# 001cat/pySurfInv

Measured on AMD Instinct MI355X. Metric: layered-model dispersion forward solves/sec (20 periods), higher is better.
Workload: dtype f32 (root search, Love group velocity) + f64 (Rayleigh eigenfunction state)

## Files before the change

### pysurfinv_amd/csrc/surfdisp_kernels.hip

```cpp
#include <hip/hip_runtime.h>
#include <stdint.h>
#include <type_traits>
#include <atomic>
#include "surfdisp_internal.h"

#include "surfdisp_k_common.h"
#include "surfdisp_k_prep.h"
#include "surfdisp_k_secular.h"
#include "surfdisp_k_rows.h"

namespace sd {

enum { ST_SCAN = 0, ST_REFINE = 1, ST_ELLIP = 2, ST_DONE = 3, ST_NEVILL = 4, ST_WREF = 5, ST_WEND = 6, ST_NEVILL0 = 7 };


template <int KIND, int G, bool INDEP, bool FAST = false, bool EXACT = false>
__device__ __forceinline__ void phase_body(const PhaseArgs &A)
{
    extern __shared__ float w_lds[];
    constexpr int S = SD_PHASE_BLOCK / G;
    constexpr int NFK = (KIND == 1) ? NFW_LOVE : NFW;
    constexpr int LS = lds_ls(S, NFK);
    const int tid = threadIdx.x;
#ifdef SD_WAVECLOCK
    const unsigned long long wclk0 = __builtin_amdgcn_s_memrealtime();
    const unsigned long long wcyc0 = __builtin_readcyclecounter();
    unsigned long long wcyc_eval = 0, wcyc_build = 0, wcyc_pre = 0, wpasses = 0;
    unsigned long long wsec[3] = {0, 0, 0}, wcyc_lean = 0, wn_lean = 0;
    unsigned long long wn_scan = 0, wn_refine = 0, wn_nevill = 0, wn_ellip = 0, wn_idle = 0, wtrip = 0, wlanelayers = 0, wlanes = 0;
#endif
    const int lane = tid & 63;
    const int slot = tid / G;
    const int j = tid % G;
    const int tbase = lane - j;
    const unsigned long long tmask =
        (G == 64) ? ~0ull : (((1ull << (G & 63)) - 1ull) << tbase);
    const int Lcap = A.Lmax, B = A.B, P = A.P;
    long tg = (long)blockIdx.x * S + slot;
    bool team_valid = INDEP ? (tg < (long)B * P) : (tg < B);
    if (EXACT) {
        team_valid = tg < (long)(*A.fb_count);
        tg = team_valid ? (long)A.fb_list[tg] : 0;
    }
    const int b = INDEP ? (int)(tg % B) : (int)tg;
    const int k_own = INDEP ? (int)(tg / B) : 0;
    float *wq = w_lds + slot;
    constexpr bool ELL_HERE = EXACT || (G < 4);
    const bool want_ratio = ELL_HERE && (KIND == 2) && (A.ratio != nullptr);
    constexpr bool OVERLAP = false;
    float *nvx = w_lds + (size_t)((!EXACT && G >= 4 && A.overlap != 0) ? 2 : 1) * LS * Lcap + (size_t)slot * 24, *nvy = nvx + 12;
    const float *__restrict__ mrow = A.msrc + (size_t)b * A.ms_b;
    const size_t msf = (size_t)A.ms_f, msi = (size_t)A.ms_i;
#define M_AT(f, i) mrow[(size_t)(f) * msf + (size_t)(i) * msi]

    int n = 0, st = ST_DONE;
    if (team_valid) { n = A.nl[b]; if (n >= 2) st = ST_SCAN; }

    int k = k_own, nsolved = 0, mm_carry = n, mm_frozen = n, sub = 0, passes = 0;
    int nflat_cur = n;
    float T = 1.0f, b1top = 0.0f;
    float p0c = 0.0f, p0d = 0.0f;
    float cb = 0.0f, db = 0.0f;
    float croot = 0.0f, r12 = 0.0f;
    int p0mm = 0;
    bool p0ok = false;
    bool first = true;
    int status = SURFDISP_OK;
    constexpr int FSTRIDE = (FAST && G <= 4) ? SD_CERT_STRIDE : 4;
    static_assert(!(FAST && EXACT), "the exact fallback walks every grid point");
    constexpr bool CERT = FAST && (G >= 2) && (G <= 8);
    int p0Kp = 0x40000000;
    bool coarse = false;
    int fine_left = 1;
    float q0c = 0.0f, q0d = 0.0f; int q0mm = 0; [[maybe_unused]] bool q0ok = false;
    [[maybe_unused]] float p0phi = 0.0f;
    bool ell_pend = false;
    int nv_nev = 1, nv_m = 1, nv_ic = 0;
    bool defer = false;
    bool ell_flag = false;
    const float ell_c2min = (want_ratio && !EXACT && team_valid && A.ovf != nullptr && A.ell_ambig != 0.0f)
                                ? __expf(0.25f * A.ovf[2 * (size_t)B + b]) / A.ell_gmax : 0.0f;

    auto build = [&](int nflat) {
        const float lnT = logf(1.0f / T);
        for (int i = j; i < nflat; i += G) {
            const bool hs = (i == nflat - 1);
            LayerRaw r;
            r.a_ref = M_AT(F_VP, i); r.b_ref = M_AT(F_VS, i); r.rho_ref = M_AT(F_RHO, i);
            r.qs = M_AT(F_QS, i);
            r.dif = hs ? 0.0f : M_AT(F_DIF, i); r.qqq = hs ? 0.0f : M_AT(F_QQQ, i);
            r.dfl = hs ? 0.0f : M_AT(F_DFL, i);
            r.hsf = hs ? M_AT(F_HSF, i) : 0.0f; r.hsr = hs ? M_AT(F_HSR, i) : 0.0f;
            const LayerV v = layer_derive(r, lnT, hs);
            W_B(i) = v.b; W_R(i) = v.rho; W_D(i) = v.d;
            if (KIND == 1 && !EXACT) W_IR(i) = wk_ilove(v.rho, v.b);
            else if (i == 0 || EXACT) W_IR(i) = wk_irho(v.rho);
            if (KIND == 2) {
                W_IA2(i) = EXACT ? v.a : wk_ia2(v.a);
                W_IB2(i) = wk_ib2(v.b);
            }
        }
        if (KIND == 2 && !EXACT) {
            __builtin_amdgcn_wave_barrier();
            __builtin_amdgcn_fence(__ATOMIC_RELEASE, "wavefront");
            __builtin_amdgcn_fence(__ATOMIC_ACQUIRE, "wavefront");
            const int top = nflat < n ? nflat : n - 1;
            for (int i = 1 + j; i <= top; i += G) W_IR(i) = wk_rat(W_R(i - 1), W_R(i));
        }
        __builtin_amdgcn_wave_barrier();
        __builtin_amdgcn_fence(__ATOMIC_RELEASE, "wavefront");
        __builtin_amdgcn_fence(__ATOMIC_ACQUIRE, "wavefront");
    };

    float dtot = 0.0f;
    auto bracket_phase = [&](float c1, float c2, int mm) -> float {
        const float om = 6.2831853f * __builtin_amdgcn_rcpf(T);
        const float i1 = __builtin_amdgcn_rcpf(c1 * c1), i2 = __builtin_amdgcn_rcpf(c2 * c2);
        const float sq = 1.001f * om * sqrt_hw(fmaxf(i1 - i2, 0.0f));
        if (sq * dtot * ((KIND == 2) ? 2.0f : 1.0f) <= A.phimulti) return 0.0f;
        float dosc = 0.0f;
        for (int i = j; i < mm - 1; i += G) {
            const float d = W_D(i);
            if (KIND == 2) dosc += ((W_IB2(i) > i2) ? d : 0.0f) + ((W_IA2(i) > i2) ? d : 0.0f);
            else           dosc += (W_B(i) < c2) ? d : 0.0f;
        }
#pragma unroll
        for (int d = G >> 1; d > 0; d >>= 1) dosc += __shfl_xor(dosc, d);
        if (sq * dosc <= A.phimulti) return 0.0f;
        float sum = 0.0f;
        for (int i = j; i < mm - 1; i += G) {
            const float od = om * W_D(i);
            const float ib2 = (KIND == 2) ? W_IB2(i) : W_IR(i) * W_R(i);
            sum += od * (sqrt_hw(fmaxf(ib2 - i2, 0.0f)) - sqrt_hw(fmaxf(ib2 - i1, 0.0f)));
            if (KIND == 2) {
                const float ia2 = W_IA2(i);
                sum += od * (sqrt_hw(fmaxf(ia2 - i2, 0.0f)) - sqrt_hw(fmaxf(ia2 - i1, 0.0f)));
            }
        }
#pragma unroll
        for (int d = G >> 1; d > 0; d >>= 1) sum += __shfl_xor(sum, d);
        return fabsf(sum);
    };

    auto entry_overflow_risk = [&](float c_lo) -> bool {
        if (EXACT || !team_valid) return false;
        if (KIND == 1) {
            const float bb = W_B(0);
            if (!(bb > c_lo)) return !(c_lo > 0.0f && T > 0.0f);
            const float q0 = 6.2831853f * __builtin_amdgcn_rcpf(c_lo * T) * W_D(0) *
                             sqrt_hw(fmaxf(1.0f - c_lo * c_lo * __builtin_amdgcn_rcpf(bb * bb), 0.0f));
            return !(q0 < 76.0f);
        }
        const float hthick = A.ovf[b], lnrho2 = A.ovf[(size_t)B + b], lng4 = A.ovf[2 * (size_t)B + b];
        const float c_hi = W_B(mm_carry - 1) + 0.31f;
        const float lnmag = 12.566371f * hthick / (c_lo * T) + lnrho2 + 4.0f * __logf(c_hi) +
                            fmaxf(lng4 - 8.0f * __logf(c_lo), 0.0f);
        return !(lnmag < 84.0f);
    };

    bool nodrop = false;
    auto no_drop_possible = [&](float c_lo) -> bool {
        float dsum = 0.0f;
        for (int i = j; i < n; i += G) dsum += W_D(i);
#pragma unroll
        for (int d = G >> 1; d > 0; d >>= 1) dsum += __shfl_xor(dsum, d);
        dtot = dsum;
        return dsum * 1.00001f <= FACT * c_lo * T;
    };

    if (st != ST_DONE) {
        T = A.per[k];
        for (int i = j; i < Lcap; i += G) { W_IR(i) = 0.0f; W_B(i) = 0.0f; W_R(i) = 0.0f; W_D(i) = 0.0f; if (KIND == 2) { W_IA2(i) = 0.0f; W_IB2(i) = 0.0f; } }
        build(n);
        b1top = W_B(0);
        const bool water = M_AT(F_VS, 0) < 0.1f;
        const int il = water ? 1 : 0;
        const float b_corr = M_AT(F_QS, il) * logf(1.0f / T) / PI_REF;
        float qq = M_AT(F_VS, il);
        if (KIND == 2) qq = 0.9f * qq;
        p0c = qq * (1.0f + b_corr);
        if (water) p0c = 0.5f;
        first = true;
        nodrop = no_drop_possible(p0c);
        defer = (!EXACT && A.strict != 0) || entry_overflow_risk(p0c);
        if (CERT) coarse = nodrop;
    }

    int wprio = -1;
    const bool LOCK = !EXACT && (INDEP ? A.lockstep >= 2 : A.lockstep != 0);
#ifdef SD_DEBUG_TRIALS
    constexpr bool LEAN = false;
#else
    constexpr bool LEAN = !FAST && !EXACT && !INDEP && (G == 2);
#endif
#ifdef SD_NO_GUARD_HANDBACK
    constexpr bool LEAN_BHS = false;
#else
    constexpr bool LEAN_BHS = LEAN && (KIND == 2);
#endif
    auto nevill_start = [&]() {
        nv_ic = 0; nv_nev = 1; nv_m = 1;
        croot = (p0c + cb) / 2.0f;
        st = (KIND == 1 && !EXACT) ? ST_NEVILL0 : ST_NEVILL;
        sub = 0;
        if (!EXACT && j == 0 && A.amb_count) atomicAdd(A.amb_count, 1);
    };
    while (__any(st != ST_DONE)) {
#ifdef SD_WAVECLOCK
        const unsigned long long wp0 = __builtin_readcyclecounter();
#endif
        if (!INDEP && A.balance) {
            const int kw = __builtin_amdgcn_readfirstlane(k);
            const int pr = 3 - min(3, (4 * kw) / max(P, 1));
            if (pr != wprio) {
                wprio = pr;
                if (pr == 3) __builtin_amdgcn_s_setprio(3);
                else if (pr == 2) __builtin_amdgcn_s_setprio(2);
                else if (pr == 1) __builtin_amdgcn_s_setprio(1);
                else __builtin_amdgcn_s_setprio(0);
            }
        }
        const bool lean = LEAN && A.scan_general == 0 && __all(st == ST_SCAN || st == ST_WREF || st == ST_DONE);
        float cj = 1.0f;
        int mmj = 2, start = 1;
        bool eval = (st != ST_DONE) && (st != ST_WREF) && (st != ST_WEND);
        const int js = (OVERLAP && ell_pend && st == ST_SCAN) ? j - 2 : j;
        if (st == ST_SCAN) {
            const int nadd = (CERT && coarse) ? FSTRIDE * (first ? js : js + 1) : (first ? js : js + 1);
            cj = p0c;
            if (CERT) {
#pragma unroll
                for (int i = 0; i < FSTRIDE * G; ++i) if (i < nadd) cj = cj + DC;
            } else {
#pragma unroll
                for (int i = 0; i < G; ++i) if (i < nadd) cj = cj + DC;
            }
            mmj = nodrop ? (n < 2 ? 2 : n) : drop_layers(wq, LS, S, n, cj, T);
        } else if (st == ST_NEVILL0) {
            const bool hi = (G == 1) ? (sub != 0) : ((j & 1) != 0);
            cj = hi ? cb : p0c; mmj = hi ? mm_frozen : p0mm;
        } else if (st == ST_NEVILL) {
            cj = croot; mmj = mm_frozen;
        } else if (st == ST_REFINE) {
            const float w = cb - p0c;
            cj = p0c + (float)(j + 1) * (w * (1.0f / (float)(G + 1)));
            if (G <= 4 && G > 1 && p0ok && w > 16.0f * CLUSTER_DC) {
                float ts = -p0d * w * __builtin_amdgcn_rcpf(db - p0d);
                const float off = (G == 4) ? ((j == 0) ? -4.0f : (j == 1) ? -1.0f : (j == 2) ? 1.0f : 4.0f)
                                           : ((j == 0) ? -1.5f : 1.5f);
                const float half = ((G == 4) ? 4.0f : 1.5f) * CLUSTER_DC;
                ts = fminf(fmaxf(ts, half + CLUSTER_DC), w - half - CLUSTER_DC);
                if (ts == ts) cj = p0c + (ts + off * CLUSTER_DC);
            }
            mmj = mm_frozen;
        } else if (st == ST_ELLIP) {
            cj = croot; mmj = mm_frozen;
            start = (G == 1) ? 2 + sub : 2 + j;
            eval = (G == 1) || (j < 2);
        }
        float val = 0.0f, phj = 0.0f;
        int kcj = 0; bool kuncj = false;
#ifdef SD_WAVECLOCK
        const unsigned long long we0 = __builtin_readcyclecounter();
        wcyc_pre += we0 - wp0;
        ++wpasses;
        {
            const unsigned long long lead = __ballot(j == 0);
            wn_scan += __popcll(__ballot(st == ST_SCAN) & lead); wn_refine += __popcll(__ballot(st == ST_REFINE) & lead);
            wn_nevill += __popcll(__ballot(st == ST_NEVILL) & lead); wn_ellip += __popcll(__ballot(st == ST_ELLIP) & lead);
            wn_idle += __popcll(__ballot(st == ST_DONE || st == ST_WREF || st == ST_WEND) & lead);
            int mx = eval ? mmj : 0, sm = eval ? mmj : 0;
            for (int d = 32; d > 0; d >>= 1) { mx = max(mx, __shfl_xor(mx, d)); sm += __shfl_xor(sm, d); }
            wtrip += mx; wlanelayers += sm; wlanes += __popcll(__ballot(eval));
        }
#endif
        float vmag = 0.0f;
        [[maybe_unused]] float bhsj = 0.0f;
        if (eval) {
            const bool want_mag = want_ratio && st == ST_ELLIP;
            if (KIND == 2) val = EXACT ? delta_rayleigh_ref(wq, LS, S, mmj, cj, T, start)
                                       : delta_rayleigh<(G != 2) && !FAST, CERT, (G <= 16)>(wq, LS, S, mmj, cj, T, start, phj, &vmag, want_mag, &kcj, &kuncj, coarse,
                                                                                                            LEAN_BHS ? &bhsj : nullptr
#ifdef SD_WAVECLOCK
                                                                                                            , wsec
#endif
                                                                                                            );
            else if (!EXACT && (st == ST_NEVILL || st == ST_NEVILL0)) val = delta_love_ref_body(wq, LS, S, mmj, cj, T);
            else           val = EXACT ? delta_love_ref(wq, LS, S, mmj, cj, T)
                                       : delta_love<CERT, (G <= 16)>(wq, LS, S, mmj, cj, T, phj, kcj, kuncj, coarse);
        }
        const bool ell_amb = !EXACT && want_ratio && eval && st == ST_ELLIP && A.ell_ambig != 0.0f &&
                             (A.ell_ambig < 0.0f || fabsf(val) < A.ell_ambig * vmag ||
                              cj * cj < ell_c2min);
#ifdef SD_WAVECLOCK
        const unsigned long long wl0 = __builtin_readcyclecounter();
        wcyc_eval += wl0 - we0;
#endif
        if (lean) {
            const bool scan = (st == ST_SCAN);
            auto negnan = [](float x) { return signbit(x) && !(x != x); };
            float oc = cj, od = val; int omm = mmj;
            float sc = p0c, sv_ = p0d; int smm = p0mm;
            if (G == 2) {
                oc = pair_swap(cj); od = pair_swap(val); omm = pair_swap(mmj);
                sc = oc; sv_ = od; smm = omm;
            } else if (G > 2) {
                const int lm1 = (lane + 63) & 63;
                sc = __shfl(cj, lm1); sv_ = __shfl(val, lm1); smm = __shfl(mmj, lm1);
            }
            const float pc = (j == 0) ? p0c : sc, pd = (j == 0) ? p0d : sv_;
            const int pmm = (j == 0) ? p0mm : smm;
            const bool has_prev = !(first && j == 0);
            const bool cross = has_prev && (negnan(val) != negnan(pd));
            bool guard = false;
            if (scan && has_prev && !cross) {
                if constexpr (LEAN_BHS) guard = (cj < 0.8f * b1top) || !(cj < bhsj + 0.3f);
                else                    guard = (cj < 0.8f * b1top) || !(cj < W_B(mmj - 1) + 0.3f);
            }
            const unsigned long long em = __ballot(scan && (cross || guard)) & tmask;
            const int fl = em ? (__ffsll((long long)em) - 1) : -1;
            const int q = (fl < 0) ? tbase + G - 1 : fl;
            const bool q_cross = ((__ballot(cross) >> q) & 1ull) != 0ull;
            float q_c, q_d, q_pc, q_pd;
            int q_mm, q_pmm;
            if (G == 1) {
                q_c = cj; q_d = val; q_mm = mmj; q_pc = pc; q_pd = pd; q_pmm = pmm;
            } else if (G == 2) {
                const bool mine = (q == lane), q_lo = (q == tbase);
                q_c = mine ? cj : oc; q_d = mine ? val : od; q_mm = mine ? mmj : omm;
                q_pc = q_lo ? p0c : ((j == 0) ? cj : oc);
                q_pd = q_lo ? p0d : ((j == 0) ? val : od);
                q_pmm = q_lo ? p0mm : ((j == 0) ? mmj : omm);
            } else {
                q_c = __shfl(cj, q); q_d = __shfl(val, q); q_mm = __shfl(mmj, q);
                q_pc = __shfl(pc, q); q_pd = __shfl(pd, q); q_pmm = __shfl(pmm, q);
            }
            if (scan && ((__ballot(scan && !fin(val)) & tmask) != 0ull)) defer = true;
            bool failed = false;
            if (scan) {
                ++passes;
                if (fl >= 0 && q_cross) {
                    p0c = q_pc; p0d = q_pd; cb = q_c; db = q_d; mm_frozen = q_mm; p0mm = q_pmm;
                    p0ok = (q_pmm == q_mm);
                    passes = 0;
                    st = LOCK ? ST_WREF : ST_REFINE;
                    if (!LOCK && bracket_phase(p0c, cb, mm_frozen) > A.phimulti) nevill_start();
                } else if (fl >= 0) {
                    failed = true;
                } else {
                    p0c = q_c; p0d = q_d; p0mm = q_mm; first = false;
                    if (passes > 100000) failed = true;
                }
            }
            if (defer) {
                if (j == 0) A.fb_list[atomicAdd(A.fb_count, 1)] = (int)tg;
                defer = false; st = ST_DONE; failed = false;
            }
            if (failed) {
                status = (k == 0) ? SURFDISP_NOROOT : SURFDISP_PARTIAL;
                st = ST_DONE;
            }
            if (LOCK && !__any(st == ST_SCAN) && st == ST_WREF) {
                st = ST_REFINE;
                if (bracket_phase(p0c, cb, mm_frozen) > A.phimulti) nevill_start();
            }
#ifdef SD_WAVECLOCK
            wcyc_lean += __builtin_readcyclecounter() - wl0; ++wn_lean;
#endif
            continue;
        }
        const int lm1 = (lane + 63) & 63;
        const float sc = __shfl(cj, lm1), sv_ = __shfl(val, lm1);
        const float pc = (j == 0) ? p0c : sc;
        const float pd = (j == 0) ? p0d : sv_;
        const int smm = __shfl(mmj, lm1);
        const int pmm = (j == 0) ? p0mm : smm;
        const int kpk = CERT ? ((kcj + 4096) | (kuncj ? 0x40000000 : 0)) : 0;
        const int sKp = CERT ? __shfl(kpk, lm1) : 0;
        const int pKp = (j == 0) ? p0Kp : sKp;
        const bool searching = ((st == ST_SCAN) || (st == ST_REFINE)) ;
        const bool has_prev = !((st == ST_SCAN) && first && (js == 0));
        auto negnan = [](float x) { return signbit(x) && !(x != x); };
        const bool cross = has_prev && (negnan(val) != negnan(pd));
#ifdef SD_DEBUG_TRIALS
        if (A.B == 1 && eval && k == SD_DEBUG_TRIALS && cj > SD_DEBUG_CMIN)
            printf("k %d pass %d st %d lane %d c %.7f val % .6e mm %d count %d unsafe %d coarse %d | p0c %.7f p0d % .4e cb %.7f db % .4e\n", k, passes, st, j, cj, val, mmj, kcj, (int)kuncj, (int)coarse, p0c, p0d, cb, db);
#endif
        bool guard = false;
        if (st == ST_SCAN && has_prev && !cross)
            guard = (cj < 0.8f * b1top) || !(cj < W_B(mmj - 1) + 0.3f);
        bool uncert = false, back0 = false;
        if (CERT) {
            if (coarse && st == ST_SCAN) {
                const bool near_hs = !(cj < W_B(mmj - 1) - 2.0f * (float)FSTRIDE * DC);
                const bool low_guard = (pc + DC) < 0.8f * b1top;
                uncert = has_prev && (near_hs || low_guard || !((pmm == mmj) && fin(pd) && fin(val) && !kuncj && (pKp == kpk)));
            }
        }
        const bool ev = searching && (cross || guard || uncert);
        const unsigned long long em = __ballot(ev) & tmask;
        const int fl = em ? (__ffsll((long long)em) - 1) : -1;
        const int src = (fl < 0) ? tbase : fl;
        const float e_c = __shfl(cj, src), e_d = __shfl(val, src);
        const float e_pc = __shfl(pc, src), e_pd = __shfl(pd, src);
        const int e_mm = __shfl(mmj, src);
        const int e_pmm = __shfl(pmm, src);
        const int l_mm = __shfl(mmj, tbase + G - 1);
        const int e_cross = __shfl((int)cross, src);
        const int t_back0 = CERT ? __shfl((int)back0, tbase) : 0;
        const int lastl = tbase + G - 1;
        const float l_c = __shfl(cj, lastl), l_d = __shfl(val, lastl);
        const float l_phi = CERT ? __shfl(phj, lastl) : 0.0f;
        const int l_Kp = CERT ? __shfl(kpk, lastl) : 0;
        const int e_pKp = CERT ? __shfl(pKp, src) : 0;
        float v0 = 0.0f, v1 = 0.0f;
        if (__any((st == ST_ELLIP) | (st == ST_NEVILL) | (st == ST_NEVILL0))) { v0 = __shfl(val, tbase); v1 = __shfl(val, (G > 1) ? tbase + 1 : tbase); }
        float e_nc = 0.0f, e_nd = 0.0f, pl_c = 0.0f, pl_d = 0.0f, e_ppc = 0.0f, e_ppd = 0.0f, e_n2c = 0.0f, e_n2d = 0.0f,
              pl2_c = 0.0f, pl2_d = 0.0f;
        int pl_mm = 0;
        if (CERT || __any(st == ST_REFINE)) {
            const int nxt = (src < lastl) ? src + 1 : lastl;
            e_nc = __shfl(cj, nxt); e_nd = __shfl(val, nxt);
            const int pl = (G > 1) ? lastl - 1 : lastl;
            pl_c = __shfl(cj, pl); pl_d = __shfl(val, pl);
            if (CERT) pl_mm = __shfl(mmj, pl);
            const int lm2s = (src - 2 >= tbase) ? src - 2 : tbase;
            e_ppc = __shfl(cj, lm2s); e_ppd = __shfl(val, lm2s);
            const int nx2 = (src + 2 <= lastl) ? src + 2 : lastl;
            e_n2c = __shfl(cj, nx2); e_n2d = __shfl(val, nx2);
            const int pl2 = (G > 2) ? lastl - 2 : lastl;
            pl2_c = __shfl(cj, pl2); pl2_d = __shfl(val, pl2);
        }
        const bool had_ell = OVERLAP && ell_pend && (st == ST_SCAN);

        bool solved = false, failed = false;
        bool fatal = false, multi = false;
        if (!EXACT) {
            const bool nonfin = ((__ballot(eval && !fin(val)) & tmask) != 0ull);
            if (st != ST_DONE && nonfin) defer = true;
            if (st == ST_REFINE && passes == 0) {
                const int ncross = __popcll(__ballot(searching && cross) & tmask) + ((negnan(l_d) != negnan(db)) ? 1 : 0);
                multi = ncross >= 2;
            }
        }
        if (CERT && st == ST_SCAN && coarse) {
            ++passes;
            if (fl >= 0) {
                p0c = e_pc; p0d = e_pd; p0mm = e_pmm;
                if (CERT) p0Kp = e_pKp;
                const bool e_back = (fl == tbase) && (t_back0 != 0);
                if (e_back) { p0c = q0c; p0d = q0d; p0mm = q0mm; }
                coarse = false; fine_left = (e_cross && !e_back) ? FSTRIDE : 2 * FSTRIDE; q0ok = false;
                if (CERT) { fine_left = FSTRIDE; first = false; }
            } else {
                q0c = pl_c; q0d = pl_d; q0mm = pl_mm; q0ok = true;
                p0c = l_c; p0d = l_d; p0mm = l_mm; p0phi = l_phi;
                if (CERT) { p0Kp = l_Kp; first = false; }
            }
        } else if (st == ST_SCAN) {
            ++passes;
            if (fl >= 0 && e_cross) {
                p0c = e_pc; p0d = e_pd; cb = e_c; db = e_d; mm_frozen = e_mm; p0mm = e_pmm;
                p0ok = (e_pmm == e_mm);
                passes = 0;
                st = LOCK ? ST_WREF : ST_REFINE;
                if (EXACT || (!LOCK && bracket_phase(p0c, cb, mm_frozen) > A.phimulti)) nevill_start();
            } else if (fl >= 0) {
                failed = true;
            } else {
                p0c = l_c; p0d = l_d; p0mm = l_mm; first = false;
                if (CERT) p0Kp = l_Kp;
                if (CERT) { p0phi = l_phi; q0d = pl_d; q0mm = pl_mm; }
                if (passes > 100000) failed = true;
                if (CERT) {
                    fine_left -= had_ell ? G - 2 : G;
                    if (fine_left <= 0 && nodrop) { coarse = true; q0ok = false; }
                    if (CERT && coarse) first = true;
                }
            }
        } else if (!EXACT && st == ST_REFINE && multi) {
            nv_ic = 0; nv_nev = 1; nv_m = 1;
            croot = (p0c + cb) / 2.0f;
            st = (KIND == 1) ? ST_NEVILL0 : ST_NEVILL;
            sub = 0;
        } else if (st == ST_NEVILL0) {
            if (G == 1) { if (sub == 0) { p0d = val; sub = 1; } else { db = val; st = ST_NEVILL; } }
            else { p0d = v0; db = v1; st = ST_NEVILL; }
        } else if (st == ST_NEVILL) {
#pragma clang fp contract(off)
            auto sg = [](float x) { return (signbit(x) && !(x != x)) ? -1.0f : 1.0f; };
            auto sgsub = [&](float a, float bq) {
                const float r = a - bq;
                if (r != r) return ((a != a) || (bq != bq)) ? 1.0f : -1.0f;
                return signbit(r) ? -1.0f : 1.0f;
            };
            float c1 = p0c, c2 = cb, d1 = p0d, d2 = db, c3 = croot;
            const float d3 = v0;
            nv_ic = nv_ic + 1;
            bool fin_ = false;
            if (!(nv_ic < 50)) fatal = true;
            else {
                bool bis;
                if (c1 - c3 <= 0.0f) bis = (c2 - c3 <= 0.0f);
                else bis = !(c2 - c3 < 0.0f);
                if (!bis) {
                    const float s13s = sgsub(d1, d3), s32s = sgsub(d3, d2);
                    if (sg(d3) * sg(d1) <= 0.0f) { c2 = c3; d2 = d3; } else { c1 = c3; d1 = d3; }
                    if (fabsf(c1 - c2) - 0.1e-5f <= 0.0f) fin_ = true;
                    else {
                        if (s13s != s32s) nv_nev = 0;
                        const float ss1 = fabsf(d1), s1 = 0.1f * ss1, ss2 = fabsf(d2), s2 = 0.1f * ss2;
                        if (s1 > ss2 || s2 > ss1) bis = true;
                        else if (nv_nev == 0) bis = true;
                        else {
                            int m = nv_m;
                            if (nv_nev == 2) { nvx[m + 1] = c3; nvy[m + 1] = d3; }
                            else { nvx[1] = c1; nvy[1] = d1; nvx[2] = c2; nvy[2] = d2; m = 1; }
                            const float ym1 = nvy[m + 1];
                            for (int kk = 1; kk <= m; ++kk) {
                                const int jn = m - kk + 1;
                                const float yj = nvy[jn];
                                if (fabsf(ym1 - yj) <= 0.1e-7f) { bis = true; break; }
                                nvx[jn] = (-yj * nvx[jn + 1] + ym1 * nvx[jn]) / (ym1 - yj);
                            }
                            if (!bis) { c3 = nvx[1]; nv_nev = 2; nv_m = (m + 1 > 10) ? 10 : m + 1; }
                        }
                    }
                }
                if (!fin_ && bis) { c3 = (c1 + c2) / 2.0f; nv_nev = 1; nv_m = 1; }
                p0c = c1; p0d = d1; cb = c2; db = d2; croot = c3;
            }
            if (fin_) {
                if (croot <= W_B(mm_frozen - 1)) {
                    if (want_ratio) { st = ST_ELLIP; sub = 0; } else solved = true;
                } else failed = true;
            }
        } else if (st == ST_REFINE) {
            float tc, td;
            bool tok = true;
            float uc = 0.0f, ud = 0.0f;
            bool uok = false;
            const float oa = p0c, oda = p0d, ob = cb, odb = db;
            const bool oaok = p0ok;
            if (fl >= 0) {
                if (fl != tbase) p0ok = true;
                p0c = e_pc; p0d = e_pd; cb = e_c; db = e_d;
                if (fl < lastl) { tc = e_nc; td = e_nd; } else { tc = ob; td = odb; }
                if (fl >= tbase + 2) { uc = e_ppc; ud = e_ppd; uok = true; }
                else if (fl == tbase + 1) { uc = oa; ud = oda; uok = oaok; }
                else if (fl + 2 <= lastl) { uc = e_n2c; ud = e_n2d; uok = true; }
                else if (fl + 1 == lastl) { uc = ob; ud = odb; uok = true; }
            } else {
                p0c = l_c; p0d = l_d; p0ok = true;
                if (G > 1) { tc = pl_c; td = pl_d; } else { tc = oa; td = oda; tok = oaok; }
                if (G > 2) { uc = pl2_c; ud = pl2_d; uok = true; }
            }
            {
                const float w = cb - p0c, sx = tc - p0c;
                const float fm = fmaxf(fabsf(p0d), fabsf(db));
                const int fex = (fm > 0.0f && fin(fm)) ? __builtin_amdgcn_frexp_expf(fm) : 0;
                const float f0 = ldexpf(p0d, -fex), f1 = ldexpf(db, -fex), f2 = ldexpf(td, -fex);
                ud = ldexpf(ud, -fex);
                auto qt = [](float a, float bq) { return a * __builtin_amdgcn_rcpf(bq); };
                float ts = qt(-f0 * w, f1 - f0);
                float t = qt(w * (f0 * f2), (f1 - f0) * (f1 - f2)) + qt(sx * (f0 * f1), (f2 - f0) * (f2 - f1));
                if (!(ts >= 0.0f)) ts = 0.0f;
                if (!(ts <= w)) ts = w;
                if (!p0ok) ts = 0.5f * w;
                const bool inside = p0ok && tok && (t >= 0.0f) && (t <= w);
                auto bends = [&](float xs, float fs) {
                    const float dm = f1 - f0;
                    const float dn = (xs > w) ? fs - f1 : f0 - fs, hn = (xs > w) ? xs - w : 0.0f - xs;
                    return !(fabsf(dn * w - dm * hn) <= 0.25f * fabsf(dm * hn));
                };
                const bool smooth = inside && !bends(sx, f2);
                bool agree = smooth && (fabsf(t - ts) <= A.atol);
                if (smooth && !agree && uok && !bends(uc - p0c, ud)) {
                    const float sx2 = uc - p0c, f3 = ud;
                    const float t2 = qt(w * (f0 * f3), (f1 - f0) * (f1 - f3)) + qt(sx2 * (f0 * f1), (f3 - f0) * (f3 - f1));
                    agree = (t2 >= 0.0f) && (t2 <= w) && (fabsf(t - t2) <= A.atol);
                }
                ++passes;
                bool accept = !(w > 1.0e-6f) || passes > 64;
                if (!accept && !(w > A.wtol) && agree) {
                    accept = !(W_B(mm_frozen - 1) <= cb * 1.000001f);
#ifdef SD_COUNT_KINK
                    if (j == 0 && A.amb_count && !accept) atomicAdd(A.amb_count + 1, 1);
#endif
                }
                if (accept) {
                    croot = p0c + (inside ? t : ts);
                    if (p0c >= 16.0f) fatal = true;
                    else if (croot <= W_B(mm_frozen - 1)) {
                        if (want_ratio) { st = ST_ELLIP; sub = 0; } else solved = true;
                    } else failed = true;
                }
            }
        } else if (st == ST_ELLIP) {
            if ((__ballot(ell_amb) & tmask) != 0ull) ell_flag = true;
            if (G == 1) {
                if (sub == 0) { r12 = val; sub = 1; }
                else { r12 = 0.5f * val / r12; solved = true; }
            } else {
                r12 = 0.5f * v1 / v0;
                solved = true;
            }
        }
        if (!EXACT && defer) {
            if (j == 0) A.fb_list[atomicAdd(A.fb_count, 1)] = (int)tg;
            defer = false; st = ST_DONE; solved = false; failed = false; fatal = false;
        }
        if (fatal) {
            nsolved = 0; k = 0; status = SURFDISP_NUMERIC; st = ST_DONE; ell_pend = false; solved = false; failed = false;
        }
        if (failed) {
            status = (k == 0) ? SURFDISP_NOROOT : SURFDISP_PARTIAL;
            st = ST_DONE;
        }
        if (LOCK) {
            if (solved) { st = ST_WEND; solved = false; }
            if (!__any(st == ST_SCAN) && st == ST_WREF) {
                st = ST_REFINE;
                if (bracket_phase(p0c, cb, mm_frozen) > A.phimulti) nevill_start();
            }
            if (!__any(st == ST_SCAN || st == ST_WREF || st == ST_REFINE || st == ST_NEVILL || st == ST_NEVILL0 || st == ST_ELLIP) && st == ST_WEND)
                solved = true;
        }
#ifdef SD_WAVECLOCK
        const unsigned long long wb0 = __builtin_readcyclecounter();
#endif
        if (solved) {
            if (j == 0) {
                A.c[(size_t)k * B + b] = croot;
                if (want_ratio) A.ratio[(size_t)k * B + b] = r12;
                if (A.hist) A.hist[(size_t)k * B + b] = EXACT ? (int)(0x80000000u | (unsigned)nflat_cur | ((unsigned)mm_frozen << 16))
                                                              : (nflat_cur | (mm_frozen << 16) | (ell_flag ? 0x40000000 : 0));
            }
            ell_flag = false;
            nsolved = ++k;
            if (INDEP || k >= P) { st = ST_DONE; }
            else {
                T = A.per[k];
                mm_carry = mm_frozen;
#ifdef SD_DEBUG_TRIALS
                if (A.B == 1 && j == 0) printf("period %d starts: previous root %.7f, layers rebuilt for T = %.4f: %d of %d\n", k, croot, T, mm_carry, n);
#endif
                build(mm_carry);
                nflat_cur = mm_carry;
                b1top = W_B(0);
                p0c = 0.90f * croot;
                p0d = 0.0f; p0mm = 0; p0ok = false; first = true; passes = 0;
                coarse = false; fine_left = 1; q0ok = false;
                st = ST_SCAN;
                nodrop = no_drop_possible(p0c);
                defer = entry_overflow_risk(p0c);
                if (CERT) coarse = nodrop;
            }
        }
#ifdef SD_WAVECLOCK
        wcyc_build += __builtin_readcyclecounter() - wb0;
#endif
    }
#ifdef SD_WAVECLOCK
    if (!EXACT && A.wclk && (threadIdx.x & 63) == 0) {
        const size_t w = (size_t)blockIdx.x * (SD_PHASE_BLOCK / 64) + (threadIdx.x >> 6);
        unsigned long long *o = A.wclk + 24 * w;
        o[0] = wclk0; o[1] = __builtin_amdgcn_s_memrealtime();
        o[2] = __builtin_readcyclecounter() - wcyc0; o[3] = wcyc_eval;
        o[4] = wcyc_build; o[5] = wpasses; o[6] = wcyc_pre;
        o[7] = wn_scan; o[8] = wn_refine; o[9] = wn_nevill; o[10] = wn_ellip; o[11] = wn_idle;
        o[12] = wtrip; o[13] = wlanelayers; o[14] = wlanes; o[15] = wsec[0];
        o[16] = wsec[1]; o[17] = wsec[2]; o[18] = wcyc_lean; o[19] = wn_lean;
    }
#endif
    if (INDEP) {
        if (team_valid && j == 0 && n >= 2 && status != SURFDISP_OK) {
            A.c[(size_t)k_own * B + b] = 0.0f;
            atomicMin(&A.nsolved[b], status == SURFDISP_NUMERIC ? -1 : k_own);
        }
        return;
    }
    if (team_valid && j == 0) {
        if (n < 2) status = SURFDISP_BADMODEL;
        for (int q = nsolved; q < P; ++q) A.c[(size_t)q * B + b] = 0.0f;
        A.nsolved[b] = nsolved;
        if (A.status) A.status[b] = status;
    }
#undef M_AT
}

template <int KIND, int G, bool INDEP, bool FAST = false, bool EXACT = false>
__global__ __launch_bounds__(SD_PHASE_BLOCK) void surfdisp_phase_kernel(PhaseArgs A)
{
    phase_body<KIND, G, INDEP, FAST, EXACT>(A);
}

__global__ __launch_bounds__(256) void surfdisp_ellip_kernel(EllipArgs A)
{
    const size_t idx = (size_t)blockIdx.x * blockDim.x + threadIdx.x;
    const int B = A.B, P = A.P;
    if (idx >= (size_t)B * P) return;
    const int b = (int)(idx % B), k = (int)(idx / B);
    const int n = A.nl[b];
    if (n < 2 || k >= A.nsolved[b]) return;
    const int hk = A.hist[idx];
    if (hk < 0) return;
    if (A.only_flagged && !(hk & 0x40000000)) return;
    const int mmf = (hk >> 16) & 0x3fff;
    const size_t fs = (size_t)A.Lmax * B;
    const float c = A.c[idx], T = A.per[k];
    struct Replay { int kk, nflat; float lnT; };
    const Replay r0{k, hk & 0xffff, logf(1.0f / T)};
    auto layer = [&](int i, Replay &r) -> LayerV {
        while (r.nflat <= i && r.kk > 0) {
            --r.kk;
            const int h = A.hist[(size_t)r.kk * B + b];
            r.nflat = (h < 0) ? n : (h & 0xffff);
            r.lnT = logf(1.0f / A.per[r.kk]);
        }
        return layer_derive(layer_load(A.mdl, fs, (size_t)i * B + b), r.lnT, i == r.nflat - 1);
    };
    const int last = mmf - 1;
    float v2 = 0.0f, v3 = 0.0f;
    bool exact = A.only_flagged != 0;
    if (!exact) {
        const RTrial t = ray_trial(c, T);
        int kk = k;
        int nflat = hk & 0xffff;
        float lnT = r0.lnT;
        RState s2{}, s3{};
        float phi = 0.0f, rho_prev = 0.0f;
        RLyr y{};
        float rho_i = 0.0f;
        for (int i = 0; i <= last; ++i) {
            while (nflat <= i && kk > 0) {
                --kk;
                const int h = A.hist[(size_t)kk * B + b];
                nflat = (h < 0) ? n : (h & 0xffff);
                lnT = logf(1.0f / A.per[kk]);
            }
            const LayerV v = layer_derive(layer_load(A.mdl, fs, (size_t)i * B + b), lnT, i == nflat - 1);
            rho_prev = rho_i;
            rho_i = v.rho;
            y.sv = v.b; y.d = v.d;
            y.ia2 = wk_ia2(v.a);
            y.ib2 = wk_ib2(v.b);
            y.rat = (i > 0) ? wk_rat(rho_prev, rho_i) : 0.0f;
            if (i == 0) {
                const float irho0 = wk_irho(rho_i);
                s2 = ray_start(t, 2, irho0);
                s3 = ray_start(t, 3, irho0);
                if (last >= 1) { ray_step<true>(s2, t, y, 2, phi); ray_step<true>(s3, t, y, 3, phi); }
            } else if (i < last) {
                ray_step<false>(s2, t, y, 2, phi);
                ray_step<false>(s3, t, y, 3, phi);
            }
        }
        const float rp = (last >= 1) ? rho_prev : 0.0f;
        float m2 = 0.0f, m3 = 0.0f;
        v2 = ray_close(s2, t, y, rho_i, rp, 2, &m2); v3 = ray_close(s3, t, y, rho_i, rp, 3, &m3);
        const float b2max = A.ovf ? 0.5f * __expf(0.25f * A.ovf[2 * (size_t)B + b]) : 0.0f;
        exact = (A.ell_ambig < 0.0f) ||
                ((A.ell_ambig > 0.0f) && (fabsf(v2) < A.ell_ambig * m2 || fabsf(v3) < A.ell_ambig * m3 || 2.0f * b2max > A.ell_gmax * c * c));
    }
    if (exact) {
        Replay r = r0;
        v2 = delta_rayleigh_ref_gen([&](int m) { const LayerV v = layer(m, r); return RefLyr{v.a, v.b, v.rho, v.d}; }, mmf, c, T, 2);
        r = r0;
        v3 = delta_rayleigh_ref_gen([&](int m) { const LayerV v = layer(m, r); return RefLyr{v.a, v.b, v.rho, v.d}; }, mmf, c, T, 3);
        if (A.amb_count) atomicAdd(A.amb_count + 1, 1);
    }
    A.ratio[idx] = 0.5f * v3 / v2;
}

struct Drop { int hs_layer; int nreg_hs; };

template <int KIND>
SD_HD __forceinline__ Drop drop_group(const float *__restrict__ mdl, size_t fs, int B, int b,
                                           int n, float lnT, float c, float T, int ndiv, bool water,
                                           float div)
{
    const float dmax = FACT * T * c;
    float sum = 0.0f;
    Drop r; r.hs_layer = n - 1; r.nreg_hs = 0;
    LayerRaw nraw = layer_load(mdl, fs, (size_t)b);
    for (int jl = 0; jl < n; ++jl) {
        const LayerRaw raw = nraw;
        if (jl + 1 < n) nraw = layer_load(mdl, fs, (size_t)(jl + 1) * B + b);
        const LayerV v = layer_derive(raw, lnT, jl == n - 1);
        if (!(c < v.b)) continue;
        if (jl == n - 1) break;
        const int nsub = (jl == 0 && water) ? 1 : ndiv;
        const float dsub = (ndiv > 1 && !(jl == 0 && water)) ? v.d / div : v.d;
        for (int s = 0; s < nsub; ++s) sum = sum + dsub;
        if (!(sum > dmax)) continue;
        const LayerV nx = layer_derive(nraw, lnT, jl + 1 == n - 1);
        bool lower, equal;
        if (KIND == 2) {
            lower = (nx.a < v.a) || (nx.a == v.a && nx.b < v.b);
            equal = (nx.a == v.a) && (nx.b == v.b);
        } else {
            lower = nx.b < v.b;
            equal = nx.b == v.b;
        }
        if (lower) { r.hs_layer = jl; r.nreg_hs = nsub - 1; break; }
        if (equal) continue;
        r.hs_layer = jl + 1; r.nreg_hs = 0; break;
    }
    return r;
}

#define SD_NO_DROP_SLACK 1.0e-4f
SD_HD __forceinline__ bool group_no_cut(const float *__restrict__ mdl, size_t fs, int B, int b, int n, float c, float T)
{
    float tot = 0.0f;
    for (int jl = 0; jl + 1 < n; ++jl) tot = tot + fabsf(mdl[F_DFL * fs + (size_t)jl * B + b]);
    return tot * (1.0f + SD_NO_DROP_SLACK) <= FACT * T * c;
}
template <int KIND>
SD_HD __forceinline__ Drop drop_or_none(const float *__restrict__ mdl, size_t fs, int B, int b,
                                             int n, float lnT, float c, float T, int ndiv, bool water,
                                             float div)
{
#ifndef SD_NO_DROP_SHORTCUT
    if (group_no_cut(mdl, fs, B, b, n, c, T)) return Drop{n - 1, 0};
#endif
    return drop_group<KIND>(mdl, fs, B, b, n, lnT, c, T, ndiv, water, div);
}

struct KOut {
    float *b;
    size_t stride;
    ptrdiff_t off_a, off_r;
    int raw;
    SD_HD void put(int i, float vb, float va, float vr) const
    {
        float *q = b + (size_t)i * stride;
        *q = vb;
        if (off_a) *reinterpret_cast<float *>(reinterpret_cast<char *>(q) + off_a) = va;
        if (off_r) *reinterpret_cast<float *>(reinterpret_cast<char *>(q) + off_r) = vr;
    }
};
struct EOut {
    float *p;
    size_t stride, plane;
    SD_HD void put(int i, float ur, float uz, float tz, float tr) const
    {
        float *q = p + (size_t)i * stride;
        q[0] = ur; q[plane] = uz; q[2 * plane] = tz; q[3 * plane] = tr;
    }
    SD_HD void put2(int i, float ut, float tq) const
    {
        float *q = p + (size_t)i * stride;
        q[0] = ut; q[plane] = tq;
    }
};
struct EUnit { float div; int hs; float i0, i1, i2; };
struct K3 { float b, a, r; };
struct Chain { float dbdb, dadb, dada, rfac; };
SD_HD __forceinline__ Chain chain_of(const LayerRaw &r, float lnT, bool is_halfspace, bool raw)
{
    if (raw) return Chain{1.0f, 0.0f, 1.0f, 1.0f};
    const float qsq = r.qs * lnT / PI_REF;
    const float qpq = qsq * 1.33333333f * (r.b_ref * r.b_ref) / (r.a_ref * r.a_ref);
    const float vfac = is_halfspace ? r.hsf : r.dif;
    Chain ch;
    ch.dbdb = (1.0f + qsq) * vfac;
    ch.dadb = 2.66666667f * qsq * (r.b_ref / r.a_ref) * vfac;
    ch.dada = (1.0f - qpq) * vfac;
    ch.rfac = is_halfspace ? r.hsr : r.qqq;
    return ch;
}
struct KC { float b1, b2, a, r; };
SD_HD __forceinline__ KC kern_coef(const LayerRaw &raw, const LayerV &v, float lnT, bool is_halfspace, float cw, bool rawc)
{
    const Chain ch = chain_of(raw, lnT, is_halfspace, rawc);
    const float rc2 = 2.0f * v.rho * cw;
    return KC{rc2 * v.b * ch.dbdb, rc2 * v.a * ch.dadb, rc2 * v.a * ch.dada, cw * ch.rfac / v.rho};
}
typedef double KR;
SD_HD __forceinline__ K3 kern_layer_rayleigh(const KC &kc, float rho, float xlamb, float xmu, float wvno, float wvnosq,
                                             float omegsq, KR dmmr, KR dmmz, KR drsz, KR dzsr, KR smmz, KR smmr)
{
    const KR two = 2, k2 = wvnosq, tk = 2.0f * wvno;
    const KR dldl = -k2 * dmmr + tk * drsz - smmz;
    const KR dldm = -k2 * (two * dmmr + dmmz) - tk * dzsr - (two * smmz + smmr);
    const KR dldr = (KR)omegsq * (dmmr + dmmz);
    return K3{(float)((KR)kc.b1 * (dldm - two * dldl) + (KR)kc.b2 * dldl), (float)((KR)kc.a * dldl),
              (float)((KR)kc.r * ((KR)rho * dldr + (KR)xlamb * dldl + (KR)xmu * dldm))};
}

struct RCoef { float a12, a13, a21, a24, a31, a34, a42, a43, ddz; };

struct RInt {
    double i0, i1, i2;
};

struct M2x2 { double a, b, c, d; };
SD_HD __forceinline__ M2x2 mm(const M2x2 &x, const M2x2 &y)
{
#pragma clang fp contract(off)
    M2x2 r;
    r.a = fma(x.a, y.a, x.b * y.c); r.b = fma(x.a, y.b, x.b * y.d);
    r.c = fma(x.c, y.a, x.d * y.c); r.d = fma(x.c, y.b, x.d * y.d);
    return r;
}
SD_HD __forceinline__ M2x2 mm2(const M2x2 &x, const M2x2 &y, const M2x2 &u, const M2x2 &v)
{
#pragma clang fp contract(off)
    M2x2 r;
    r.a = fma(x.a, y.a, fma(x.b, y.c, fma(u.a, v.a, u.b * v.c))); r.b = fma(x.a, y.b, fma(x.b, y.d, fma(u.a, v.b, u.b * v.d)));
    r.c = fma(x.c, y.a, fma(x.d, y.c, fma(u.c, v.a, u.d * v.c))); r.d = fma(x.c, y.b, fma(x.d, y.d, fma(u.c, v.b, u.d * v.d)));
    return r;
}
SD_HD __forceinline__ M2x2 madd(const M2x2 &x, const M2x2 &y)
{
    M2x2 r; r.a = x.a + y.a; r.b = x.b + y.b; r.c = x.c + y.c; r.d = x.d + y.d; return r;
}
struct RProp { M2x2 p11, p12, p21, p22; };

SD_HD __forceinline__ RProp make_prop(const RCoef &q)
{
#pragma clang fp contract(off)
    const double wh = (double)(0.5f * q.ddz), w1 = (double)(1.0f * q.ddz);
    const double t6 = (double)((1.0f / 6.0f) * q.ddz), t3 = (double)((1.0f / 3.0f) * q.ddz);
    const double k1 = (t6 + t3) + (t3 + t6);
    const double k2 = (t3 * wh + t3 * wh) + t6 * w1;
    const double k3 = t3 * wh * wh + t6 * w1 * wh;
    const double k4 = t6 * w1 * wh * wh;
    const M2x2 m1 = {(double)q.a31, (double)q.a34, (double)q.a21, (double)q.a24};
    const M2x2 m2 = {(double)q.a13, (double)q.a12, (double)q.a43, (double)q.a42};
    RProp P;
    auto diag_block = [&](const M2x2 &nn) -> M2x2 {
        const double tr = nn.a + nn.d;
        const double det = fma(nn.a, nn.d, -(nn.b * nn.c));
        const double al = fma(k4, tr, k2), be = fma(-k4, det, 1.0);
        return M2x2{fma(al, nn.a, be), al * nn.b, al * nn.c, fma(al, nn.d, be)};
    };
    auto off_block = [&](const M2x2 &nn, const M2x2 &m) -> M2x2 {
        const M2x2 q = {fma(k3, nn.a, k1), k3 * nn.b, k3 * nn.c, fma(k3, nn.d, k1)};
        return mm(q, m);
    };
    {
        const M2x2 n1 = mm(m1, m2);
        P.p11 = diag_block(n1);
        P.p12 = off_block(n1, m1);
    }
    {
        const M2x2 n2 = mm(m2, m1);
        P.p22 = diag_block(n2);
        P.p21 = off_block(n2, m2);
    }
    return P;
}
struct RPow { double f0, f1, g0, g1; };
struct RBase { M2x2 m1, m2, n1, n2; double t, d; RPow p; };
SD_HD __forceinline__ RBase make_base(const RCoef &q)
{
#pragma clang fp contract(off)
    const double wh = (double)(0.5f * q.ddz), w1 = (double)(1.0f * q.ddz);
    const double t6 = (double)((1.0f / 6.0f) * q.ddz), t3 = (double)((1.0f / 3.0f) * q.ddz);
    const double k1 = (t6 + t3) + (t3 + t6);
    const double k2 = (t3 * wh + t3 * wh) + t6 * w1;
    const double k3 = t3 * wh * wh + t6 * w1 * wh;
    const double k4 = t6 * w1 * wh * wh;
    RBase r;
    r.m1 = M2x2{(double)q.a31, (double)q.a34, (double)q.a21, (double)q.a24};
    r.m2 = M2x2{(double)q.a13, (double)q.a12, (double)q.a43, (double)q.a42};
    r.n1 = mm(r.m1, r.m2);
    r.n2 = mm(r.m2, r.m1);
    r.t = r.n1.a + r.n1.d;
    r.d = fma(r.n1.a, r.n1.d, -(r.n1.b * r.n1.c));
    r.p = RPow{fma(-k4, r.d, 1.0), fma(k4, r.t, k2), k1, k3};
    return r;
}
// ... 1773 lines not shown
```

Measured before the change: 43.74 million.

## Evaluate a second scan pair per pass in lean Rayleigh scan before deciding

In the lean G=2 Rayleigh scan path, when neither lane of a pair sees a sign change, guard hit, deferral or non-finite value, the pair immediately evaluates the next two trial velocities inside the same pass. A shared four-point scan decision then updates the bracket. This amortises the per-pass bookkeeping, ballots and state-machine overhead over twice as many secular evaluations. The cost is extra evaluations past a root when only one pair in the wave continues, more divergence, and higher register pressure. The lean path is now also restricted to lockstep mode.

```diff
diff --git a/pysurfinv_amd/csrc/surfdisp_k_scan.h b/pysurfinv_amd/csrc/surfdisp_k_scan.h
--- /dev/null
+++ b/pysurfinv_amd/csrc/surfdisp_k_scan.h
@@ -0,0 +1,44 @@
+#pragma once
+#include "surfdisp_k_common.h"
+
+namespace sd {
+
+struct ScanPt {
+    float v, c;
+    int mm;
+    bool g;
+};
+
+struct ScanOut {
+    int e;
+    bool cross;
+    ScanPt lo;
+    ScanPt hi;
+};
+
+SD_HD __forceinline__ bool scan_negnan(float x) { return __builtin_signbit(x) && !(x != x); }
+
+SD_HD __forceinline__ bool scan_event(float prev_v, bool has_prev, float v, bool g, bool *cross)
+{
+    *cross = has_prev && (scan_negnan(v) != scan_negnan(prev_v));
+    return *cross || (has_prev && g);
+}
+
+template <int N>
+SD_HD __forceinline__ ScanOut scan_decide(const ScanPt &p0, const bool first, const ScanPt (&pt)[N])
+{
+    ScanOut o;
+    o.e = -1; o.cross = false; o.lo = pt[N - 1]; o.hi = pt[N - 1];
+#pragma unroll
+    for (int i = N - 1; i >= 0; --i) {
+        const ScanPt &pv = (i > 0) ? pt[i > 0 ? i - 1 : 0] : p0;
+        bool cr;
+        if (scan_event(pv.v, (i > 0) || !first, pt[i].v, pt[i].g, &cr)) { o.e = i; o.cross = cr; o.lo = pv; o.hi = pt[i]; }
+    }
+    return o;
+}
+
+SD_HD __forceinline__ ScanOut scan_decide2(const ScanPt &p0, const bool first, const ScanPt (&pt)[2]) { return scan_decide<2>(p0, first, pt); }
+SD_HD __forceinline__ ScanOut scan_decide4(const ScanPt &p0, const bool first, const ScanPt (&pt)[4]) { return scan_decide<4>(p0, first, pt); }
+
+}
diff --git a/pysurfinv_amd/csrc/surfdisp_kernels.hip b/pysurfinv_amd/csrc/surfdisp_kernels.hip
--- a/pysurfinv_amd/csrc/surfdisp_kernels.hip
+++ b/pysurfinv_amd/csrc/surfdisp_kernels.hip
@@ -7,6 +7,7 @@
 #include "surfdisp_k_common.h"
 #include "surfdisp_k_prep.h"
 #include "surfdisp_k_secular.h"
+#include "surfdisp_k_scan.h"
 #include "surfdisp_k_rows.h"
 
 namespace sd {
@@ -26,7 +27,7 @@
     const unsigned long long wclk0 = __builtin_amdgcn_s_memrealtime();
     const unsigned long long wcyc0 = __builtin_readcyclecounter();
     unsigned long long wcyc_eval = 0, wcyc_build = 0, wcyc_pre = 0, wpasses = 0;
-    unsigned long long wsec[3] = {0, 0, 0}, wcyc_lean = 0, wn_lean = 0;
+    unsigned long long wsec[3] = {0, 0, 0}, wcyc_lean = 0, wn_lean = 0, wn_double = 0;
     unsigned long long wn_scan = 0, wn_refine = 0, wn_nevill = 0, wn_ellip = 0, wn_idle = 0, wtrip = 0, wlanelayers = 0, wlanes = 0;
 #endif
     const int lane = tid & 63;
@@ -198,6 +199,11 @@
 #else
     constexpr bool LEAN_BHS = LEAN && (KIND == 2);
 #endif
+#ifdef SD_NO_DOUBLE_SCAN
+    constexpr bool LEAN2 = false;
+#else
+    constexpr bool LEAN2 = LEAN_BHS;
+#endif
     auto nevill_start = [&]() {
         nv_ic = 0; nv_nev = 1; nv_m = 1;
         croot = (p0c + cb) / 2.0f;
@@ -220,7 +226,7 @@
                 else __builtin_amdgcn_s_setprio(0);
             }
         }
-        const bool lean = LEAN && A.scan_general == 0 && __all(st == ST_SCAN || st == ST_WREF || st == ST_DONE);
+        const bool lean = LEAN && A.scan_general == 0 && (!LEAN2 || LOCK) && __all(st == ST_SCAN || st == ST_WREF || st == ST_DONE);
         float cj = 1.0f;
         int mmj = 2, start = 1;
         bool eval = (st != ST_DONE) && (st != ST_WREF) && (st != ST_WEND);
@@ -261,10 +267,10 @@
         float val = 0.0f, phj = 0.0f;
         int kcj = 0; bool kuncj = false;
 #ifdef SD_WAVECLOCK
-        const unsigned long long we0 = __builtin_readcyclecounter();
+        unsigned long long we0 = __builtin_readcyclecounter();
         wcyc_pre += we0 - wp0;
         ++wpasses;
-        {
+        auto wcount = [&]() {
             const unsigned long long lead = __ballot(j == 0);
             wn_scan += __popcll(__ballot(st == ST_SCAN) & lead); wn_refine += __popcll(__ballot(st == ST_REFINE) & lead);
             wn_nevill += __popcll(__ballot(st == ST_NEVILL) & lead); wn_ellip += __popcll(__ballot(st == ST_ELLIP) & lead);
@@ -272,10 +278,16 @@
             int mx = eval ? mmj : 0, sm = eval ? mmj : 0;
             for (int d = 32; d > 0; d >>= 1) { mx = max(mx, __shfl_xor(mx, d)); sm += __shfl_xor(sm, d); }
             wtrip += mx; wlanelayers += sm; wlanes += __popcll(__ballot(eval));
-        }
+        };
+        wcount();
 #endif
         float vmag = 0.0f;
         [[maybe_unused]] float bhsj = 0.0f;
+        [[maybe_unused]] float a_val = 0.0f;
+        [[maybe_unused]] int a_mm = 0;
+        [[maybe_unused]] bool a_g = false, second = false;
+#pragma nounroll
+        for (;;) {
         if (eval) {
             const bool want_mag = want_ratio && st == ST_ELLIP;
             if (KIND == 2) val = EXACT ? delta_rayleigh_ref(wq, LS, S, mmj, cj, T, start)
@@ -289,6 +301,37 @@
             else           val = EXACT ? delta_love_ref(wq, LS, S, mmj, cj, T)
                                        : delta_love<CERT, (G <= 16)>(wq, LS, S, mmj, cj, T, phj, kcj, kuncj, coarse);
         }
+        if constexpr (LEAN2) {
+            if (lean && !second) {
+                const bool scan = (st == ST_SCAN);
+                const float od = pair_swap(val);
+                bool cr;
+                const bool g = (cj < 0.8f * b1top) || !(cj < bhsj + 0.3f);
+                const bool ev = scan_event((j == 0) ? p0d : od, !(first && j == 0), val, g, &cr);
+                const int hit = (int)(scan && (ev || defer || !fin(val)));
+                const bool go = scan && ((hit | pair_swap(hit)) == 0);
+                if (__any(go)) {
+#ifdef SD_WAVECLOCK
+                    const unsigned long long wa0 = __builtin_readcyclecounter();
+                    wcyc_eval += wa0 - we0;
+#endif
+                    second = true;
+                    a_val = val; a_mm = mmj; a_g = g;
+                    eval = go;
+                    cj = cj + DC; cj = cj + DC;
+                    mmj = nodrop ? (n < 2 ? 2 : n) : drop_layers(wq, LS, S, n, cj, T);
+                    val = 0.0f;
+#ifdef SD_WAVECLOCK
+                    we0 = __builtin_readcyclecounter();
+                    wcyc_pre += we0 - wa0; ++wn_double;
+                    wcount();
+#endif
+                    continue;
+                }
+            }
+        }
+        break;
+        }
         const bool ell_amb = !EXACT && want_ratio && eval && st == ST_ELLIP && A.ell_ambig != 0.0f &&
                              (A.ell_ambig < 0.0f || fabsf(val) < A.ell_ambig * vmag ||
                               cj * cj < ell_c2min);
@@ -296,7 +339,69 @@
         const unsigned long long wl0 = __builtin_readcyclecounter();
         wcyc_eval += wl0 - we0;
 #endif
-        if (lean) {
+        if constexpr (LEAN2) if (lean) {
+            const bool scan = (st == ST_SCAN);
+            const bool j0 = (j == 0);
+            const ScanPt p0 = {p0d, p0c, p0mm, false};
+            const float c0 = first ? p0c : p0c + DC, c1 = c0 + DC;
+            const float av = second ? a_val : val;
+            const int am = second ? a_mm : mmj;
+            const bool ag = second ? a_g : ((cj < 0.8f * b1top) || !(cj < bhsj + 0.3f));
+            const float oav = pair_swap(av);
+            const int oam = pair_swap(am);
+            const bool oag = pair_swap((int)ag) != 0;
+            ScanOut o;
+            bool allfin;
+            if (second) {
+                const float c2 = c1 + DC, c3 = c2 + DC;
+                const bool bg = (cj < 0.8f * b1top) || !(cj < bhsj + 0.3f);
+                const float obv = pair_swap(val);
+                const int obm = pair_swap(mmj);
+                const bool obg = pair_swap((int)bg) != 0;
+                const ScanPt pt[4] = {{j0 ? av : oav, c0, j0 ? am : oam, j0 ? ag : oag}, {j0 ? oav : av, c1, j0 ? oam : am, j0 ? oag : ag},
+                                      {j0 ? val : obv, c2, j0 ? mmj : obm, j0 ? bg : obg}, {j0 ? obv : val, c3, j0 ? obm : mmj, j0 ? obg : bg}};
+                o = scan_decide4(p0, first, pt);
+                allfin = fin(av) && fin(oav) && fin(val) && fin(obv);
+            } else {
+                const ScanPt pt[2] = {{j0 ? av : oav, c0, j0 ? am : oam, j0 ? ag : oag}, {j0 ? oav : av, c1, j0 ? oam : am, j0 ? oag : ag}};
+                o = scan_decide2(p0, first, pt);
+                allfin = fin(av) && fin(oav);
+            }
+            if (scan && !allfin) defer = true;
+            bool failed = false;
+            if (scan) {
+                if (o.e >= 0 && o.cross) {
+                    p0c = o.lo.c; p0d = o.lo.v; cb = o.hi.c; db = o.hi.v; mm_frozen = o.hi.mm; p0mm = o.lo.mm;
+                    p0ok = (o.lo.mm == o.hi.mm);
+                    if (o.e >= 2) first = false;
+                    passes = 0;
+                    st = ST_WREF;
+                } else if (o.e >= 0) {
+                    failed = true;
+                } else {
+                    p0c = o.lo.c; p0d = o.lo.v; p0mm = o.lo.mm; first = false;
+                    passes += second ? 2 : 1;
+                    if (passes > 100000) failed = true;
+                }
+            }
+            if (defer) {
+                if (j == 0) A.fb_list[atomicAdd(A.fb_count, 1)] = (int)tg;
+                defer = false; st = ST_DONE; failed = false;
+            }
+            if (failed) {
+                status = (k == 0) ? SURFDISP_NOROOT : SURFDISP_PARTIAL;
+                st = ST_DONE;
+            }
+            if (!__any(st == ST_SCAN) && st == ST_WREF) {
+                st = ST_REFINE;
+                if (bracket_phase(p0c, cb, mm_frozen) > A.phimulti) nevill_start();
+            }
+#ifdef SD_WAVECLOCK
+            wcyc_lean += __builtin_readcyclecounter() - wl0; ++wn_lean;
+#endif
+            continue;
+        }
+        if (!LEAN2 && lean) {
             const bool scan = (st == ST_SCAN);
             auto negnan = [](float x) { return signbit(x) && !(x != x); };
             float oc = cj, od = val; int omm = mmj;
@@ -670,7 +775,7 @@
         o[4] = wcyc_build; o[5] = wpasses; o[6] = wcyc_pre;
         o[7] = wn_scan; o[8] = wn_refine; o[9] = wn_nevill; o[10] = wn_ellip; o[11] = wn_idle;
         o[12] = wtrip; o[13] = wlanelayers; o[14] = wlanes; o[15] = wsec[0];
-        o[16] = wsec[1]; o[17] = wsec[2]; o[18] = wcyc_lean; o[19] = wn_lean;
+        o[16] = wsec[1]; o[17] = wsec[2]; o[18] = wcyc_lean; o[19] = wn_lean; o[20] = wn_double;
     }
 #endif
     if (INDEP) {
```

Result: faster. 44.66 million (median of 6 runs) (+2.1%).
